# RobustFieldAutonomyLab/Distributional_RL_Navigation

Hardware: AMD Instinct MI355X
Metric: env steps/sec (whole node) at 65 536 envs; IQN grad-steps/sec (higher is better)
Workload: dtype f32; 1 GPU; 65536 envs/GPU + IQN training (act K=32, 8 quantiles, replay 100000, batch 256, 1 grad step(s) every 4 vector steps); envs_per_gpu=65536, n_cores=8, n_obstacles=10, precision=f64, learner=independent, ranks_per_gpu=1, act_variant=2, taus=per_env, resets=under_next_act, launches_per_grad_step=1, ablation=False

## Files before the change

distributional_rl_navigation_amd/_capi.py:

```python
import ctypes as C
import os
import subprocess

_HERE = os.path.dirname(os.path.abspath(__file__))
LIB_PATH = os.path.join(_HERE, "libmarinenav_hip.so")

MAX_CORES, MAX_OBS, NUM_BEAMS, OBS_DIM, NUM_ACTIONS, MAX_STAGES = 8, 10, 11, 26, 9, 8
PRECISION_F64, PRECISION_MIXED = 0, 1
RESET_IN_FRONT, RESET_UNDER_ACT, RESET_OWED = 0, 1, 2
QUERY_VELOCITY_GIVEN, QUERY_VELOCITY_FROM_CURRENT = 0, 1
QUERY_FLAG_COLLISION, QUERY_FLAG_OUTSIDE, QUERY_FLAG_GOAL, QUERY_FLAG_BAD_ENV = 1, 2, 4, 128
INFO_STRINGS = ("normal", "out of boundary", "too long episode", "collision", "reach goal")


class MnParams(C.Structure):
    _fields_ = [
        ("width", C.c_double), ("height", C.c_double), ("core_r", C.c_double), ("v_rel_max", C.c_double),
        ("p", C.c_double), ("v_range", C.c_double * 2), ("obs_r_range", C.c_double * 2), ("clear_r", C.c_double),
        ("goal_dis", C.c_double), ("timestep_penalty", C.c_double), ("collision_penalty", C.c_double),
        ("goal_reward", C.c_double), ("discount", C.c_double), ("min_start_goal_dis", C.c_double),
        ("init_theta", C.c_double), ("init_speed", C.c_double), ("dt", C.c_double), ("robot_r", C.c_double),
        ("max_speed", C.c_double), ("a", C.c_double * 3), ("w", C.c_double * 3), ("sonar_range", C.c_double),
        ("sonar_angle", C.c_double), ("num_cores", C.c_int32), ("num_obs", C.c_int32),
        ("reset_start_and_goal", C.c_int32), ("random_reset_state", C.c_int32), ("set_boundary", C.c_int32),
# ... 71 lines not shown
    ("mn_reset_placement", _i32, [C.c_float, _i32, _i64, _i32, _i32, _i32]),
    ("mn_reset_done_next_act", C.c_int, [_vp, _pf, _vp, C.c_float, _i32, _i32, C.POINTER(_vp), C.POINTER(C.c_uint32), _pi32]),
    ("mn_set_reset_owed_max_rows", C.c_int, [_vp, _i32]),
    ("mn_reset_is_owed", _i32, [_vp]),
    ("mn_reset_join", C.c_int, [_vp, _vp]),
    ("mn_set_reset_under_act_max", C.c_int, [_vp, _i32, C.POINTER(C.c_int64)]),
    ("mn_debug_side_delay_us", C.c_int, [_vp, _i32]),
    ("mn_debug_read", C.c_int, [_vp, _i32, _vp, _i64]),
    ("mn_load_worlds", C.c_int, [_vp, _i32, _i32, _pi32, _pd, _pi32, _pd, _pi32, _pd, _pd, _pd, _pd, _pd, _pd, _pf, _vp]),
    ("mn_get_worlds", C.c_int, [_vp, _i32, _i32, _pi32, _pd, _pi32, _pd, _pi32, _pd, _pd, _pd, _pd, _pd, _pd]),
    ("mn_query_velocity", C.c_int, [_vp, _vp, _i32, _vp, _i64, _vp, _vp]),
    ("mn_query_observation", C.c_int, [_vp, _vp, _i32, _vp, _i32, _i64, _vp, _vp, _vp, _vp]),
    ("mn_get_state", C.c_int, [_vp, _i32, _i32, _pd, _pi32, _pi64]),
    ("mn_set_state", C.c_int, [_vp, _i32, _i32, _pd, _pi32, _pi64]),
    ("mn_state_bytes", _i64, [_vp]),
    ("mn_state_save", C.c_int, [_vp, _vp, _i64, _vp]),
    ("mn_state_load", C.c_int, [_vp, _vp, _i64, _vp]),
    ("mn_enable_obs64", C.c_int, [_vp, _i32]),
    ("mn_get_obs64", C.c_int, [_vp, _i32, _i32, _pd]),
    ("mn_get_reward64", C.c_int, [_vp, _i32, _i32, _pd]),
    ("mn_enable_trajectory", C.c_int, [_vp, _i32]),
    ("mn_get_trajectory", C.c_int, [_vp, _i32, _i32, _i32, _pd]),
    ("mn_set_trajectory_trace", C.c_int, [_vp, _vp, _i32, _i32]),
    ("mn_peek_next_double", C.c_int, [_vp, _i32, _i32, _pd]),
    ("mn_last_done_count", C.c_int, [_vp, _vp, _pi32]),
    ("mn_profile_begin", C.c_int, [_vp, _i32]),
    ("mn_profile_end", C.c_int, [_vp, _vp, _pd, _pi32]),
    ("mn_profile_reset_end", C.c_int, [_vp, _vp, _pd, _pi32]),
    ("mn_iqn_create", C.c_int, [C.POINTER(_vp)]),
    ("mn_iqn_destroy", C.c_int, [_vp]),
    ("mn_iqn_weights_changed", C.c_int, [_vp]),
    ("mn_iqn_set_variant", C.c_int, [_vp, _i32]),
    ("mn_iqn_set_greedy_rows", C.c_int, [_vp, _i32]),
    ("mn_iqn_set_grid", C.c_int, [_vp, _i32]),
    ("mn_iqn_set_tau_mode", C.c_int, [_vp, _i32]),
    ("mn_iqn_set_late_rows", C.c_int, [_vp, _vp, _vp, C.c_uint32, _i32]),
    ("mn_iqn_late_timeouts", C.c_int, [_vp, _vp, C.POINTER(C.c_uint32)]),
    ("mn_iqn_late_timeouts_peek", C.c_int, [_vp, C.POINTER(C.c_uint32)]),
    ("mn_iqn_set_late_bound_ms", C.c_int, [_vp, C.c_double]),
    ("mn_iqn_train_workspace_init", C.c_int, [_vp, _i32, _vp]),
    ("mn_iqn_train_step", C.c_int, [_vp, _vp, _vp, _vp, _vp, _i64, _vp, _vp, _vp, _vp, _vp, _vp, _vp, _vp, _vp, _vp, _vp, _vp, _vp, _vp, _i32, _i32, C.c_float, _i32,
                                    _dbl, _dbl, _dbl, _dbl, _dbl, _vp]),
    ("mn_rollout_policy", C.c_int, [_vp, _i32, _i32, _vp, _vp, _vp, _vp, _vp, _vp, _vp]),
    ("mn_planner_act", C.c_int, [_vp, _i32, _i32, _pd, _pd, _vp, _vp]),
    ("mn_rollout_iqn", C.c_int, [_vp, _vp, C.POINTER(C.c_void_p), _i32, _vp, C.c_float, _i32] + [_vp] * 10),
    ("mn_rollout_iqn_rows", C.c_int, [_vp, _vp, C.POINTER(C.c_void_p), _i32, _vp, C.c_float, _i32] + [_vp] * 12),
    ("mn_rollout_iqn_eval", C.c_int, [_vp, _vp, C.POINTER(C.c_void_p), _i32, _vp, C.c_float, _i32] + [_vp] * 14),
    ("mn_iqn_image_floats", _i32, []),
    ("mn_iqn_export_image", C.c_int, [_vp, C.POINTER(C.c_void_p), _vp, _vp]),
    ("mn_rollout_iqn_groups", C.c_int, [_vp, _vp, _i64, _i32, _i32, _i32] + [_vp] * 14),
    ("mn_rollout_dqn", C.c_int, [_vp, C.POINTER(C.c_void_p), _vp, _i32, _i32] + [_vp] * 8),
    ("mn_dqn_image_floats", C.c_int64, []),
    ("mn_dqn_export_image", C.c_int, [C.POINTER(C.c_void_p), _vp, _vp]),
    ("mn_rollout_dqn_groups", C.c_int, [_vp, _vp, _i64, _i32, _i32, _i32] + [_vp] * 8),
    ("mn_dqn_act", C.c_int, [_vp, C.POINTER(C.c_void_p), _vp, _i32, _vp, _vp, _i32, _vp]),
    ("mn_dqn_train_workspace_floats", C.c_int64, [_i32]),
    ("mn_dqn_train_step", C.c_int, [_vp] * 5 + [_i64] + [_vp] * 11 + [_i32, C.c_float] + [_dbl] * 5 + [_vp]),
    ("mn_dqn_train_steps_workspace_floats", C.c_int64, [_i32, _i32]),
    ("mn_dqn_train_steps", C.c_int, [_vp] * 5 + [_i64] + [_vp] * 11 + [_i32, _i32, C.c_float] + [_dbl] * 5 + [_vp]),
    ("mn_dqn_train_steps_parts", C.c_int, [_vp] * 5 + [_i64] + [_vp] * 11 + [_i32, _i32, C.c_float] + [_dbl] * 5 + [_i32, _vp]),
    ("mn_dqn_group_create", C.c_int, [C.POINTER(MnDqnLearner), _i32, C.POINTER(_vp)]),
    ("mn_dqn_group_destroy", C.c_int, [_vp]),
    ("mn_dqn_group_train_step", C.c_int, [_vp, _i64, _vp, _vp, _vp, _vp, _i32, C.c_float] + [_dbl] * 5 + [_vp]),
    ("mn_dqn_group_train_steps", C.c_int, [_vp, _i64, _vp, _vp, _vp, _vp, _i32, _i32, C.c_float] + [_dbl] * 5 + [_vp]),
    ("mn_iqn_group_create", C.c_int, [C.POINTER(MnIqnLearner), _i32, _i32, C.POINTER(_vp)]),
    ("mn_iqn_group_destroy", C.c_int, [_vp]),
# ... 86 lines not shown
```

distributional_rl_navigation_amd/csrc/iqn_act.hip:

```cpp
#include <hip/hip_runtime.h>
#include <stdint.h>
#include <utility>
#include <vector>

#include "marinenav_hip.h"
#include "mn_internal.h"
#include "iqn_actor_group.h"

#define MN_IQN_VARIANT_DEFAULT 2

namespace {

#include "iqn_act_common.h"
#include "iqn_act_exact.h"
#include "iqn_act_split.h"
#include "iqn_act_tiled.h"
#include "iqn_act_group.h"

using ExactKernel = decltype(&iqn_qvals_kernel<false>);
using SplitKernel = decltype(&sp::iqn_qvals_split_kernel<false>);
using TiledKernel = decltype(&sp::iqn_qvals_tiled_kernel);
struct Form {
    ExactKernel exact;
    SplitKernel split;
    TiledKernel tiled;
    int lds_floats, threads;
    const void *kernel() const { return exact ? (const void *)exact : split ? (const void *)split : (const void *)tiled; }
    size_t lds_bytes() const { return lds_floats * sizeof(float); }
};
enum { F_EXACT, F_EXACT_QUANT, F_SPLIT, F_SPLIT_LATE, F_SPLIT_ROWS, F_SPLIT_LATE_ROWS, F_SPLIT_QUANT, F_SHARED, F_SHARED_QUANT, F_TILED, N_FORMS };
const Form FORMS[N_FORMS] = {
    {iqn_qvals_kernel<false>, nullptr, nullptr, LDS_FLOATS, 512},
    {iqn_qvals_kernel<true>, nullptr, nullptr, LDS_FLOATS, 512},
    {nullptr, sp::iqn_qvals_split_kernel<false>, nullptr, sp::LDS_ACT_FLOATS, 512},
    {nullptr, sp::iqn_qvals_split_kernel<false, false, sp::WAVES, true>, nullptr, sp::LDS_ACT_FLOATS, 512},
    {nullptr, sp::iqn_qvals_split_kernel<false, false, sp::WAVES, false, true>, nullptr, sp::LDS_ACT_FLOATS, 512},
    {nullptr, sp::iqn_qvals_split_kernel<false, false, sp::WAVES, true, true>, nullptr, sp::LDS_ACT_FLOATS, 512},
    {nullptr, sp::iqn_qvals_split_kernel<true>, nullptr, sp::LDS_FLOATS, 512},
    {nullptr, sp::iqn_qvals_split_kernel<false, true, 8>, nullptr, sp::OFF_FB, 512},
    {nullptr, sp::iqn_qvals_split_kernel<true, true, 8>, nullptr, sp::OFF_FB, 512},
    {nullptr, nullptr, sp::iqn_qvals_tiled_kernel, sp::TL_FLOATS, 512},
};

bool load_weights(const float *const *p, IqnWeights *w) {
    if (!p) return false;
    for (int i = 0; i < 14; ++i) if (!p[i]) return false;
    *w = {p[0], p[1], p[2], p[3], p[4], p[5], p[6], p[7], p[8], p[9], p[10], p[11], p[12], p[13]};
    return true;
}

}

struct mn_iqn_ctx {
    int device = -1;
    int n_cu = 0;
    float *packed = nullptr;
    uint32_t *packed_sp = nullptr;
    float *consts_sp = nullptr;
    float *h1_sp = nullptr;
    uint32_t *timg = nullptr;
    float *taux = nullptr;
    template <class Fn> void each_buffer(Fn f) {
        f(packed, OFF_FB); f(packed_sp, sp::OFF_FB); f(consts_sp, sp::N_CONST_BUF); f(h1_sp, sp::H1_FLOATS + 32); f(timg, sp::T_WORDS); f(taux, sp::TA_FLOATS);
    }
    int tau_mode = 0;
    bool dirty = true, dirty_sp = true;
    int variant = MN_IQN_VARIANT_DEFAULT;
    int max_blocks = 0;
    sp::LateRows late = {};
    uint32_t *late_status = nullptr;
    volatile uint32_t *late_status_host = nullptr;
    uint32_t *late_status_host_dev = nullptr;
    uint64_t late_bound_ticks = sp::LATE_BOUND_TICKS;
    std::vector<hipEvent_t> ev;
    int prof_max = 0, prof_n = 0;
    uint32_t *rollout_words = nullptr;
    bool greedy_rows = true;
    uint32_t *rows_buf = nullptr;
    int rows_cap = 0;
};

extern "C" int mn_iqn_set_grid(mn_iqn_ctx *c, int32_t max_workgroups) {
    if (!c || max_workgroups < 0) return MN_ERR_INVALID;
    c->max_blocks = max_workgroups;
    return MN_OK;
}

extern "C" int mn_iqn_create(mn_iqn_ctx **out) {
    if (!out) return MN_ERR_INVALID;
    int dev = 0;
    if (hipGetDevice(&dev) != hipSuccess) return MN_ERR_NO_DEVICE;
    hipDeviceProp_t prop;
    if (hipGetDeviceProperties(&prop, dev) != hipSuccess) return MN_ERR_HIP;
    for (const Form &f : FORMS)
        if (hipFuncSetAttribute(f.kernel(), hipFuncAttributeMaxDynamicSharedMemorySize, (int)f.lds_bytes()) != hipSuccess) return MN_ERR_HIP;
    mn_iqn_ctx *c = new mn_iqn_ctx();
    c->device = dev;
    c->n_cu = prop.multiProcessorCount;
    bool ok = true;
    c->each_buffer([&](auto *&p, size_t count) { ok = ok && hipMalloc(reinterpret_cast<void **>(&p), count * sizeof(*p)) == hipSuccess; });
    if (!ok || hipMemset(c->consts_sp, 0, sp::N_CONST_BUF * sizeof(float)) != hipSuccess || hipDeviceSynchronize() != hipSuccess) {
        c->each_buffer([](auto *p, size_t) { (void)hipFree(p); });
        delete c;
        return MN_ERR_ALLOC;
    }
    *out = c;
    return MN_OK;
}

extern "C" int mn_iqn_destroy(mn_iqn_ctx *c) {
    if (!c) return MN_ERR_INVALID;
    int cur = -1;
    const bool moved = hipGetDevice(&cur) == hipSuccess && cur != c->device;
    if (moved) (void)hipSetDevice(c->device);
    for (hipEvent_t e : c->ev) (void)hipEventDestroy(e);
    c->each_buffer([](auto *p, size_t) { (void)hipFree(p); });
    (void)hipFree(c->late_status);
    (void)hipFree(c->rollout_words);
    (void)hipFree(c->rows_buf);
    if (c->late_status_host) (void)hipHostFree((void *)c->late_status_host);
    if (moved) (void)hipSetDevice(cur);
    delete c;
    return MN_OK;
}

extern "C" int mn_iqn_weights_changed(mn_iqn_ctx *c) {
    if (!c) return MN_ERR_INVALID;
    c->dirty = true;
    c->dirty_sp = true;
    return MN_OK;
}

extern "C" int mn_iqn_set_variant(mn_iqn_ctx *c, int32_t variant) {
    if (!c || (variant != 0 && variant != 2)) return MN_ERR_INVALID;
    c->variant = variant;
    return MN_OK;
}

extern "C" int mn_iqn_set_greedy_rows(mn_iqn_ctx *c, int32_t on) {
    if (!c) return MN_ERR_INVALID;
    c->greedy_rows = on != 0;
    return MN_OK;
}

static int greedy_rows_buffer(mn_iqn_ctx *c, int n, GreedyRows *out) {
    if (n > c->rows_cap) {
        uint32_t *buf = nullptr;
        if (hipMalloc(reinterpret_cast<void **>(&buf), (4 + (size_t)n) * sizeof(uint32_t)) != hipSuccess) return MN_ERR_ALLOC;
        if (hipMemset(buf, 0, 4 * sizeof(uint32_t)) != hipSuccess || hipDeviceSynchronize() != hipSuccess) { (void)hipFree(buf); return MN_ERR_HIP; }
        (void)hipFree(c->rows_buf);
        c->rows_buf = buf;
        c->rows_cap = n;
    }
    *out = GreedyRows{reinterpret_cast<int32_t *>(c->rows_buf + 4), c->rows_buf};
    return MN_OK;
}

extern "C" int mn_iqn_last_greedy_rows(mn_iqn_ctx *c, void *stream, int32_t *list_host, int32_t cap, int32_t *count_out) {
    if (!c || !count_out || cap < 0 || (cap > 0 && !list_host)) return MN_ERR_INVALID;
    *count_out = 0;
    if (!c->rows_buf) return MN_OK;
    if (hipStreamSynchronize((hipStream_t)stream) != hipSuccess) return MN_ERR_HIP;
    uint32_t w[4];
    if (hipMemcpy(w, c->rows_buf, sizeof(w), hipMemcpyDeviceToHost) != hipSuccess) return MN_ERR_HIP;
    const uint32_t count = w[w[2] & 1u];
    if (count > (uint32_t)c->rows_cap) return MN_ERR_HIP;
    *count_out = (int32_t)count;
    const uint32_t k = count < (uint32_t)cap ? count : (uint32_t)cap;
    if (k && hipMemcpy(list_host, c->rows_buf + 4, k * sizeof(int32_t), hipMemcpyDeviceToHost) != hipSuccess) return MN_ERR_HIP;
    return MN_OK;
}

extern "C" int mn_iqn_set_tau_mode(mn_iqn_ctx *c, int32_t mode) {
    if (!c || mode < 0 || mode > 3) return MN_ERR_INVALID;
    c->tau_mode = mode;
    return MN_OK;
}

extern "C" int mn_iqn_profile_begin(mn_iqn_ctx *c, int32_t max_launches) {
    if (!c || max_launches < 0 || max_launches > 65536) return MN_ERR_INVALID;
    while ((int)c->ev.size() < 2 * max_launches) {
        hipEvent_t e;
        if (hipEventCreate(&e) != hipSuccess) return MN_ERR_HIP;
        c->ev.push_back(e);
    }
    c->prof_max = max_launches;
    c->prof_n = 0;
    return MN_OK;
}

extern "C" int mn_iqn_profile_end(mn_iqn_ctx *c, void *stream, double *mean_ms, int32_t *launches) {
    if (!c) return MN_ERR_INVALID;
    if (hipStreamSynchronize((hipStream_t)stream) != hipSuccess) return MN_ERR_HIP;
    double sum = 0.0;
    for (int i = 0; i < c->prof_n; ++i) {
        float ms = 0.f;
        if (hipEventElapsedTime(&ms, c->ev[2 * i], c->ev[2 * i + 1]) != hipSuccess) return MN_ERR_HIP;
        sum += ms;
    }
    if (mean_ms) *mean_ms = c->prof_n ? sum / c->prof_n : 0.0;
    if (launches) *launches = c->prof_n;
    c->prof_max = 0;
    c->prof_n = 0;
    return MN_OK;
}

static int act_grid(const mn_iqn_ctx *c, int n) {
    const int blocks = (n + 7) / 8, cap = c->max_blocks > 0 ? c->max_blocks : c->n_cu;
    return blocks < cap ? blocks : cap;
}

static int draw_blocks(const mn_iqn_ctx *c, long items) {
    const long blocks = (items + 255) / 256;
    return blocks < 8L * c->n_cu ? (int)blocks : 8 * c->n_cu;
}

static bool late_rows_supported(const mn_iqn_ctx *c, int n, bool quantiles) {
    if (c->variant != 2 || c->tau_mode != 0 || quantiles || n <= 0) return false;
    return (long)n <= 64L * 8L * act_grid(c, n);
}

extern "C" int mn_iqn_set_late_rows(mn_iqn_ctx *c, const uint8_t *mask_dev, const uint32_t *flags_dev, uint32_t tick, int32_t n) {
    if (!c) return MN_ERR_INVALID;
    c->late = sp::LateRows{};
    if (!mask_dev && !flags_dev) return MN_OK;
    if (!mask_dev || !flags_dev) return MN_ERR_INVALID;
    if (!late_rows_supported(c, n, false)) return 1;
    if (!c->late_status) {
        uint32_t *st = nullptr;
        void *hp = nullptr, *hd = nullptr;
        if (hipMalloc(reinterpret_cast<void **>(&st), sizeof(uint32_t)) != hipSuccess) return MN_ERR_ALLOC;
        if (hipMemset(st, 0, sizeof(uint32_t)) != hipSuccess || hipHostMalloc(&hp, sizeof(uint32_t), hipHostMallocMapped) != hipSuccess) { (void)hipFree(st); return MN_ERR_ALLOC; }
        *(volatile uint32_t *)hp = 0u;
        if (hipHostGetDevicePointer(&hd, hp, 0) != hipSuccess) { (void)hipFree(st); (void)hipHostFree(hp); return MN_ERR_HIP; }
        c->late_status = st; c->late_status_host = (volatile uint32_t *)hp; c->late_status_host_dev = (uint32_t *)hd;
    }
    c->late = sp::LateRows{mask_dev, flags_dev, tick, c->late_status, c->late_status_host_dev, c->late_bound_ticks};
    return MN_OK;
}

extern "C" int mn_iqn_late_timeouts(mn_iqn_ctx *c, void *stream, uint32_t *out) {
    if (!c || !out) return MN_ERR_INVALID;
// ... 71 lines not shown
    const bool prof = c->prof_n < c->prof_max;
    if (prof) (void)hipEventRecord(c->ev[2 * c->prof_n], s);

    const int pack_blocks = begin_pack(c, w, s);
    if (shared) {
        const int rng_blocks = rng ? draw_blocks(c, (long)n + K_TAUS) : 0;
        hipLaunchKernelGGL(sp::iqn_shared_prep_kernel, dim3(pack_blocks + sp::H1_BLOCKS + rng_blocks), dim3(256), 0, s, w, (const float *)c->consts_sp,
                           c->packed_sp, (const uint64_t *)rng_state_dev, draws_dev, n, rng ? nullptr : taus_dev, cvar, pack_blocks, c->h1_sp);
        if (rng) explore_u_dev = eps > 0.f ? draws_dev + K_TAUS : nullptr;
        taus_dev = nullptr;
        if (f.tiled)
            hipLaunchKernelGGL(sp::iqn_tiled_prep_kernel, dim3(sp::T_PREP_BLOCKS + sp::TA_PREP_BLOCKS), dim3(256), 0, s, w, (const float *)c->consts_sp,
                               (const float *)c->h1_sp, c->timg, c->taux);
    } else if (rng) {
        const int rng_blocks = draw_blocks(c, ((long)n * (K_TAUS + 1) + 3) / 4);
        MnOwedReset owed;
        if (fusable && env && mn_owed_reset_take(env, s, &owed))
            mn_launch_prep_reset(owed, MnPrepLaunch{weights, c->consts_sp, c->packed_sp, pack_blocks != 0, rng_state_dev, draws_dev, n, cvar_row_dev, cvar, eps,
                                                    listed ? actions_dev : nullptr, rows.list, rows.words, 32 * c->n_cu}, s);
        else if (f.split)
            hipLaunchKernelGGL(sp::iqn_split_prep_kernel, dim3(pack_blocks + rng_blocks), dim3(256), 0, s, w, (const float *)c->consts_sp,
                               c->packed_sp, (const uint64_t *)rng_state_dev, draws_dev, n, cvar_row_dev, cvar, pack_blocks, eps, listed ? actions_dev : nullptr,
                               rows);
        else
            hipLaunchKernelGGL(iqn_prep_kernel, dim3(pack_blocks + rng_blocks), dim3(256), 0, s, w, c->packed,
                               (const uint64_t *)rng_state_dev, draws_dev, n, cvar_row_dev, cvar, pack_blocks);
        taus_dev = draws_dev;
        explore_u_dev = eps > 0.f ? draws_dev + (size_t)n * K_TAUS : nullptr;
    } else if (pack_blocks) {
        pack_image(c, w, s);
    }

    const dim3 grid(act_grid(c, n)), block(f.threads);
    if (f.tiled)
        hipLaunchKernelGGL(f.tiled, dim3((n + 255) / 256), block, f.lds_bytes(), s, obs_dev, (const uint32_t *)c->packed_sp, (const uint32_t *)c->timg,
                           (const float *)c->taux, qvals_dev, explore_u_dev, eps, actions_dev, n, rng_state_dev);
    else if (f.split)
        hipLaunchKernelGGL(f.split, grid, block, f.lds_bytes(), s, obs_dev, taus_dev, (const uint32_t *)c->packed_sp, qvals_dev, explore_u_dev, eps,
                           actions_dev, n, rng_state_dev, quantiles_dev, shared ? (const float *)c->h1_sp : nullptr, late, rows);
    else
        hipLaunchKernelGGL(f.exact, grid, block, f.lds_bytes(), s, obs_dev, taus_dev, (const float *)c->packed, qvals_dev, explore_u_dev, eps,
                           actions_dev, n, rng_state_dev, quantiles_dev);

    if (prof) { (void)hipEventRecord(c->ev[2 * c->prof_n + 1], s); ++c->prof_n; }
    return hipGetLastError() == hipSuccess ? MN_OK : MN_ERR_HIP;
}

extern "C" int mn_iqn_refresh(mn_iqn_ctx *c, const float *const *weights, void *stream) {
    IqnWeights w;
    if (!c || !load_weights(weights, &w)) return MN_ERR_INVALID;
    int dev = -1;
    if (hipGetDevice(&dev) != hipSuccess || dev != c->device) return MN_ERR_INVALID;
    if (begin_pack(c, w, (hipStream_t)stream)) pack_image(c, w, (hipStream_t)stream);
    return hipGetLastError() == hipSuccess ? MN_OK : MN_ERR_HIP;
}

int mn_iqn_rollout_image(mn_iqn_ctx *c, const float *const *weights, hipStream_t s, const uint32_t **image, uint32_t **words) {
    if (!c || !weights || !image || !words || c->variant != 2 || c->tau_mode != 0) return MN_ERR_INVALID;
    if (!c->rollout_words) {
        uint32_t *w = nullptr;
        if (hipMalloc(reinterpret_cast<void **>(&w), 2 * sizeof(uint32_t)) != hipSuccess) return MN_ERR_ALLOC;
        if (hipMemset(w, 0, 2 * sizeof(uint32_t)) != hipSuccess || hipDeviceSynchronize() != hipSuccess) { (void)hipFree(w); return MN_ERR_HIP; }
        c->rollout_words = w;
    }
    const int rc = mn_iqn_refresh(c, weights, (void *)s);
    if (rc) return rc;
    *image = c->packed_sp;
// ... 147 lines not shown
```

distributional_rl_navigation_amd/iqn/fused_act.py:

```python
import ctypes as C
import weakref

import torch

from .. import _capi
from ..episodes import EPISODE_TRACES, trace_buffers

_ORDER = ("velocity_encoder", "goal_encoder", "sensor_encoder", "cos_embedding", "hidden_layer", "hidden_layer_2", "output_layer")


def _p(t):
    return C.c_void_p(t.data_ptr()) if t is not None else None


def _params(net):
    mods = net._modules
    out = []
    for name in _ORDER:
        ps = mods[name]._parameters
        out.append(ps["weight"]); out.append(ps["bias"])
    return out


class ActContext:

    def __init__(self, device):
        self.device = torch.device(device)
        h = C.c_void_p()
        with torch.cuda.device(self.device):
            rc = _capi.lib().mn_iqn_create(C.byref(h))
        if rc:
            raise _capi.MarineNavHipError(f"mn_iqn_create failed ({rc})")
        self.h = h
        self._sig = None
        self.variant = self.DEFAULT_VARIANT
        self.tau_mode = 0
        self.greedy_rows = True
        self._ptrs = (C.c_void_p * 14)()
        self._fin = weakref.finalize(self, _capi.lib().mn_iqn_destroy, h)

    def __deepcopy__(self, memo):
        return None

    def __reduce__(self):
        return (type(None), ())

    def weights(self, net):
        ps = _params(net)
        sig = tuple((t.data_ptr(), t._version) for t in ps)
        if sig != self._sig:
            for i, t in enumerate(ps):
                assert t.is_cuda and t.is_contiguous() and t.dtype == torch.float32
                self._ptrs[i] = t.data_ptr()
            self._sig = sig
            self.invalidate()
        return self._ptrs

    def invalidate(self):
        _capi.lib().mn_iqn_weights_changed(self.h)

    DEFAULT_VARIANT = 2

    def set_variant(self, variant):
        rc = _capi.lib().mn_iqn_set_variant(self.h, int(variant))
        if rc:
            raise _capi.MarineNavHipError(f"mn_iqn_set_variant failed ({rc})")
        self.variant = int(variant)

    def set_greedy_rows(self, on):
        if bool(on) == self.greedy_rows:
            return
        rc = _capi.lib().mn_iqn_set_greedy_rows(self.h, int(bool(on)))
        if rc:
            raise _capi.MarineNavHipError(f"mn_iqn_set_greedy_rows failed ({rc})")
        self.greedy_rows = bool(on)

    def set_tau_mode(self, mode):
        if int(mode) == self.tau_mode:
            return
        rc = _capi.lib().mn_iqn_set_tau_mode(self.h, int(mode))
        if rc:
            raise _capi.MarineNavHipError(f"mn_iqn_set_tau_mode failed ({rc})")
        self.tau_mode = int(mode)

    def set_grid(self, max_workgroups):
        rc = _capi.lib().mn_iqn_set_grid(self.h, int(max_workgroups))
        if rc:
            raise _capi.MarineNavHipError(f"mn_iqn_set_grid failed ({rc})")
        self.__dict__.pop("_late_ok", None)

    def refresh(self, net):
        stream = _capi.stream_ptr(self.device)
        rc = _capi.lib().mn_iqn_refresh(self.h, self.weights(net), stream)
        if rc:
            raise _capi.MarineNavHipError(f"mn_iqn_refresh failed ({rc})")

    def profile_begin(self, max_launches):
        rc = _capi.lib().mn_iqn_profile_begin(self.h, int(max_launches))
        if rc:
            raise _capi.MarineNavHipError(f"mn_iqn_profile_begin failed ({rc})")

    def profile_end(self):
        ms, nl = C.c_double(), C.c_int32()
        stream = _capi.stream_ptr(self.device)
        rc = _capi.lib().mn_iqn_profile_end(self.h, stream, C.byref(ms), C.byref(nl))
        if rc:
            raise _capi.MarineNavHipError(f"mn_iqn_profile_end failed ({rc})")
        return ms.value, nl.value
# ... 253 lines not shown
```

include/marinenav_hip.h:

```cpp
#ifndef MARINENAV_HIP_H
#define MARINENAV_HIP_H

#include <stdint.h>

#ifdef __cplusplus
extern "C" {
#endif

#define MN_MAX_CORES 8
#define MN_MAX_OBS 10
#define MN_NUM_BEAMS 11
#define MN_OBS_DIM 26
#define MN_NUM_ACTIONS 9
#define MN_MAX_STAGES 8

typedef enum mn_status {
    MN_OK = 0,
    MN_ERR_INVALID = -1,
    MN_ERR_HIP = -2,
    MN_ERR_NO_DEVICE = -3,
    MN_ERR_ALLOC = -4,
    MN_ERR_PEER = -5
} mn_status;

// ... 125 lines not shown
                         uint8_t *flags_dev, void *stream);

int mn_get_state(mn_handle *h, int32_t first_env, int32_t count, double *state, int32_t *episode_timesteps,
                 int64_t *total_timesteps);
int mn_set_state(mn_handle *h, int32_t first_env, int32_t count, const double *state,
                 const int32_t *episode_timesteps, const int64_t *total_timesteps);

int64_t mn_state_bytes(const mn_handle *h);
int mn_state_save(mn_handle *h, void *blob_dev, int64_t bytes, void *stream);
int mn_state_load(mn_handle *h, const void *blob_dev, int64_t bytes, void *stream);

int mn_enable_obs64(mn_handle *h, int32_t on);
int mn_get_obs64(mn_handle *h, int32_t first_env, int32_t count, double *out);
int mn_get_reward64(mn_handle *h, int32_t first_env, int32_t count, double *out);

int mn_enable_trajectory(mn_handle *h, int32_t max_substeps);
int mn_get_trajectory(mn_handle *h, int32_t first_env, int32_t count, int32_t n_substeps, double *out);
int mn_set_trajectory_trace(mn_handle *h, double *traj_trace_dev, int32_t n_steps, int32_t n_substeps);

int mn_peek_next_double(mn_handle *h, int32_t first_env, int32_t count, double *out);

int mn_last_done_count(mn_handle *h, void *stream, int32_t *out);

int mn_profile_begin(mn_handle *h, int32_t max_launches);
int mn_profile_reset_end(mn_handle *h, void *stream, double *mean_ms, int32_t *launches);
int mn_profile_end(mn_handle *h, void *stream, double *mean_ms, int32_t *launches);

typedef struct mn_iqn_ctx mn_iqn_ctx;
int mn_iqn_create(mn_iqn_ctx **out);
int mn_iqn_destroy(mn_iqn_ctx *c);
int mn_iqn_weights_changed(mn_iqn_ctx *c);
int mn_iqn_set_variant(mn_iqn_ctx *c, int32_t variant);
int mn_iqn_set_greedy_rows(mn_iqn_ctx *c, int32_t on);
int mn_iqn_set_tau_mode(mn_iqn_ctx *c, int32_t mode);
int mn_iqn_last_greedy_rows(mn_iqn_ctx *c, void *stream, int32_t *list_host, int32_t cap, int32_t *count_out);
int mn_iqn_set_late_rows(mn_iqn_ctx *c, const uint8_t *mask_dev, const uint32_t *flags_dev, uint32_t tick, int32_t n);
int mn_iqn_late_timeouts(mn_iqn_ctx *c, void *stream, uint32_t *out);
int mn_iqn_late_timeouts_peek(mn_iqn_ctx *c, uint32_t *out);
int mn_iqn_set_late_bound_ms(mn_iqn_ctx *c, double ms);
int mn_probe_mfma_clock(double target_ms, double *out, void *stream);
int mn_iqn_set_grid(mn_iqn_ctx *c, int32_t max_workgroups);
int mn_iqn_refresh(mn_iqn_ctx *c, const float *const *weights, void *stream);

int mn_iqn_act(mn_iqn_ctx *c, const float *obs_dev, const float *taus_dev, const float *const *weights, float *qvals_dev,
               const float *explore_u_dev, float eps, int32_t *actions_dev, float *quantiles_dev, int32_t n,
               int32_t num_taus, void *stream);

int mn_iqn_act_rng(mn_iqn_ctx *c, const float *obs_dev, const float *const *weights, uint64_t *rng_state_dev,
                   float *draws_dev, const float *cvar_row_dev, float cvar, float eps, int32_t *actions_dev,
                   float *qvals_dev, float *quantiles_dev, int32_t n, int32_t num_taus, void *stream);
int mn_iqn_act_rng_env(mn_iqn_ctx *c, mn_handle *env, const float *obs_dev, const float *const *weights, uint64_t *rng_state_dev,
                       float *draws_dev, const float *cvar_row_dev, float cvar, float eps, int32_t *actions_dev,
                       float *qvals_dev, float *quantiles_dev, int32_t n, int32_t num_taus, void *stream);
int mn_rollout_iqn(mn_handle *h, mn_iqn_ctx *ctx, const float *const *weights, int32_t n_steps, uint64_t *rng_state_dev, float cvar,
                   int32_t adaptive, float *obs_dev, float *obs_trace_dev, float *reward_trace_dev, uint8_t *done_trace_dev,
                   uint8_t *info_trace_dev, int32_t *action_trace_dev, float *cvar_trace_dev, float *q_trace_dev, int32_t *steps_run_dev,
                   void *stream);
int mn_rollout_iqn_rows(mn_handle *h, mn_iqn_ctx *ctx, const float *const *weights, int32_t n_steps, uint64_t *rng_state_dev, float cvar,
                        int32_t adaptive, const float *cvar_row_dev, const uint8_t *adaptive_row_dev, float *obs_dev, float *obs_trace_dev,
                        float *reward_trace_dev, uint8_t *done_trace_dev, uint8_t *info_trace_dev, int32_t *action_trace_dev, float *cvar_trace_dev,
                        float *q_trace_dev, int32_t *steps_run_dev, void *stream);
int mn_rollout_iqn_eval(mn_handle *h, mn_iqn_ctx *ctx, const float *const *weights, int32_t n_steps, uint64_t *rng_state_dev, float cvar,
                        int32_t adaptive, const float *cvar_row_dev, const uint8_t *adaptive_row_dev, float *obs_dev, float *obs_trace_dev,
                        float *reward_trace_dev, uint8_t *done_trace_dev, uint8_t *info_trace_dev, int32_t *action_trace_dev, float *cvar_trace_dev,
                        float *q_trace_dev, float *quantiles_trace_dev, float *taus_trace_dev, int32_t *steps_run_dev, void *stream);

// ... 164 lines not shown
```

Measured before the change: 910.5 million env steps/s.

## Add few-rows IQN act kernel with register ring-prefetched weights

Adds a separate act kernel for the greedy-rows split form, used when the expected number of greedy rows ((1-eps)*n) is at most a threshold (default 256). Each block handles one row at a time with two waves. Weight fragments stream from global memory through an eight-deep register ring that is prefetched and interleaved with the MFMA stages, instead of the full-device tiled/split path. The aim is lower latency when only a few rows need network evaluation, such as early high-epsilon exploration. The cost is a large new hand-scheduled kernel, and it only triggers at small greedy-row counts, so at 65536 envs with low eps it may rarely run.

```diff
diff --git a/distributional_rl_navigation_amd/_capi.py b/distributional_rl_navigation_amd/_capi.py
--- a/distributional_rl_navigation_amd/_capi.py
+++ b/distributional_rl_navigation_amd/_capi.py
@@ -127,6 +127,8 @@
     ("mn_iqn_weights_changed", C.c_int, [_vp]),
     ("mn_iqn_set_variant", C.c_int, [_vp, _i32]),
     ("mn_iqn_set_greedy_rows", C.c_int, [_vp, _i32]),
+    ("mn_iqn_set_few_rows_max", C.c_int, [_vp, _i32]),
+    ("mn_iqn_few_rows_launches", C.c_int, [_vp, C.POINTER(C.c_int64)]),
     ("mn_iqn_set_grid", C.c_int, [_vp, _i32]),
     ("mn_iqn_set_tau_mode", C.c_int, [_vp, _i32]),
     ("mn_iqn_set_late_rows", C.c_int, [_vp, _vp, _vp, C.c_uint32, _i32]),
diff --git a/distributional_rl_navigation_amd/csrc/iqn_act.hip b/distributional_rl_navigation_amd/csrc/iqn_act.hip
--- a/distributional_rl_navigation_amd/csrc/iqn_act.hip
+++ b/distributional_rl_navigation_amd/csrc/iqn_act.hip
@@ -14,6 +14,7 @@
 #include "iqn_act_common.h"
 #include "iqn_act_exact.h"
 #include "iqn_act_split.h"
+#include "iqn_act_few.h"
 #include "iqn_act_tiled.h"
 #include "iqn_act_group.h"
 
@@ -78,6 +79,8 @@
     bool greedy_rows = true;
     uint32_t *rows_buf = nullptr;
     int rows_cap = 0;
+    int few_rows_max = MN_IQN_FEW_ROWS_MAX_DEFAULT;
+    int64_t few_launches = 0;
 };
 
 extern "C" int mn_iqn_set_grid(mn_iqn_ctx *c, int32_t max_workgroups) {
@@ -143,6 +146,18 @@
     return MN_OK;
 }
 
+extern "C" int mn_iqn_set_few_rows_max(mn_iqn_ctx *c, int32_t rows) {
+    if (!c) return MN_ERR_INVALID;
+    c->few_rows_max = rows;
+    return MN_OK;
+}
+
+extern "C" int mn_iqn_few_rows_launches(mn_iqn_ctx *c, int64_t *out) {
+    if (!c || !out) return MN_ERR_INVALID;
+    *out = c->few_launches;
+    return MN_OK;
+}
+
 static int greedy_rows_buffer(mn_iqn_ctx *c, int n, GreedyRows *out) {
     if (n > c->rows_cap) {
         uint32_t *buf = nullptr;
@@ -208,6 +223,17 @@
 static int act_grid(const mn_iqn_ctx *c, int n) {
     const int blocks = (n + 7) / 8, cap = c->max_blocks > 0 ? c->max_blocks : c->n_cu;
     return blocks < cap ? blocks : cap;
+}
+
+static bool few_rows(const mn_iqn_ctx *c, const Form &f, int n, float eps) {
+    if (&f != &FORMS[F_SPLIT_ROWS] || c->few_rows_max < 0) return false;
+    return (1.0 - (eps < 1.f ? (double)eps : 1.0)) * (double)n <= (double)c->few_rows_max;
+}
+
+static int few_grid(const mn_iqn_ctx *c, int n) {
+    const int cap = c->max_blocks > 0 ? c->max_blocks : c->n_cu, want = c->few_rows_max < 1 ? 1 : c->few_rows_max;
+    const int blocks = want < cap ? want : cap;
+    return blocks < n ? blocks : n;
 }
 
 static int draw_blocks(const mn_iqn_ctx *c, long items) {
@@ -345,7 +371,11 @@
     }
 
     const dim3 grid(act_grid(c, n)), block(f.threads);
-    if (f.tiled)
+    if (few_rows(c, f, n, eps)) {
+        ++c->few_launches;
+        hipLaunchKernelGGL(sp::iqn_act_few_kernel, dim3(few_grid(c, n)), dim3(64 * sp::FEW_WAVES), 0, s, obs_dev, taus_dev, (const uint32_t *)c->packed_sp, actions_dev,
+                           n, rng_state_dev, rows);
+    } else if (f.tiled)
         hipLaunchKernelGGL(f.tiled, dim3((n + 255) / 256), block, f.lds_bytes(), s, obs_dev, (const uint32_t *)c->packed_sp, (const uint32_t *)c->timg,
                            (const float *)c->taux, qvals_dev, explore_u_dev, eps, actions_dev, n, rng_state_dev);
     else if (f.split)
diff --git a/distributional_rl_navigation_amd/csrc/iqn_act_few.h b/distributional_rl_navigation_amd/csrc/iqn_act_few.h
--- /dev/null
+++ b/distributional_rl_navigation_amd/csrc/iqn_act_few.h
@@ -0,0 +1,294 @@
+
+namespace sp {
+
+constexpr int FEW_WAVES = 2;
+constexpr int FEW_DEPTH = 8;
+constexpr int FEW_PRE = 4;
+constexpr int FEW_MID = 4;
+
+constexpr int FEW_L1 = 0, FEW_L2 = 1, FEW_B2 = 2, FEW_L3 = 3, FEW_B3 = 4, FEW_W4 = 5;
+struct FewGrp { int kind, a, b; };
+constexpr FewGrp few_group(int gi) {
+    int k = 0;
+    for (int t = 0; t < 4; ++t, ++k) if (k == gi) return {FEW_L1, t, 0};
+    for (int B = 0; B < KB2 - 1; ++B) {
+        for (int h = 0; h < 2; ++h, ++k) if (k == gi) return {FEW_L2, B, h};
+        for (int t = 2 * B + 4; t < 2 * B + 6 && t < T1; ++t, ++k) if (k == gi) return {FEW_L1, t, 0};
+    }
+    for (int h = 0; h < 2; ++h, ++k) if (k == gi) return {FEW_L2, KB2 - 1, h};
+    if (k++ == gi) return {FEW_B2, 0, 0};
+    for (int kb = 0; kb < 2; ++kb)
+        for (int h = 0; h < 2; ++h, ++k) if (k == gi) return {FEW_L3, kb, h};
+    if (k++ == gi) return {FEW_B3, 0, 0};
+    if (k++ == gi) return {FEW_W4, 0, 0};
+    return {-1, 0, 0};
+}
+constexpr int few_index(int kind, int a, int b) {
+    for (int gi = 0; gi < 64; ++gi) {
+        const FewGrp g = few_group(gi);
+        if (g.kind < 0) break;
+        if (g.kind == kind && g.a == a && g.b == b) return gi;
+    }
+    return -1;
+}
+constexpr int FEW_GROUPS = few_index(FEW_W4, 0, 0) + 1;
+static_assert(FEW_GROUPS == T1 + 2 * KB2 + 4 + 3, "every weight operand of a row once, and the three groups of f32 constants");
+constexpr int few_unit(int gi, int j) {
+    const FewGrp g = few_group(gi);
+    if (g.kind == FEW_L1) return j < 4 ? W1_U4 + (4 * g.a + j) * 64 : (OFF_B1 >> 2) + 4 * g.a;
+    if (g.kind == FEW_L2) return W2_U4 + (((2 * g.b + (j >> 1)) * KB2 + g.a) * 2 + (j & 1)) * 64;
+    if (g.kind == FEW_L3) return W3_U4 + (((2 * g.b + (j >> 1)) * 2 + g.a) * 2 + (j & 1)) * 64;
+    if (g.kind == FEW_B2) return (OFF_B2 >> 2) + 4 * j;
+    if (g.kind == FEW_B3) return (OFF_B3 >> 2) + 4 * j;
+    return (OFF_W4 >> 2) + j * 64;
+}
+static_assert(OFF_B1 % 4 == 0 && OFF_B2 % 4 == 0 && OFF_B3 % 4 == 0 && OFF_W4 % 4 == 0, "16-byte aligned blocks");
+
+typedef u32x4 FewRing[FEW_DEPTH][5];
+
+typedef const __attribute__((address_space(1))) char *FewImage;
+struct FewOff { uint32_t lane, group; FewImage image; };
+__device__ __forceinline__ u32x4 few_ld(const FewOff &o, int unit, uint32_t off) {
+    return *reinterpret_cast<const __attribute__((address_space(1))) u32x4 *>(o.image + 16 * unit + off);
+}
+template <int GI>
+__device__ __forceinline__ void few_load(FewRing &ring, const FewOff &o) {
+    if constexpr (GI < FEW_GROUPS) {
+        constexpr FewGrp G = few_group(GI);
+        constexpr int s = GI % FEW_DEPTH;
+        constexpr bool by_group = G.kind == FEW_B2 || G.kind == FEW_B3;
+        static_for<4>([&](auto J_) {
+            constexpr int j = decltype(J_)::value;
+            ring[s][j] = few_ld(o, few_unit(GI, j), by_group ? o.group : o.lane);
+        });
+        if constexpr (G.kind == FEW_L1) ring[s][4] = few_ld(o, few_unit(GI, 4), o.group);
+    }
+}
+
+template <int B>
+__device__ __forceinline__ void few_stage(FewRing &ring, const FewOff &o, const f32x4 *__restrict__ fbv,
+                                          const f16x8 (&cbh)[2], const f16x8 (&cbl)[2], const f16x8 bh, const f16x8 bl, f32x4 (&acc2)[4],
+                                          f32x4 (&accW)[2], const f32x4 (&accR)[2], f16x8 &bhN, f16x8 &blN) {
+    constexpr int NTI_W = (B + 2 < KB2) ? ntiles_of(B + 2) : 0;
+    constexpr int NTI_R = (B + 1 >= 0 && B + 1 < KB2) ? ntiles_of(B + 1) : 0;
+    constexpr int N_L2 = B >= 0 ? 12 : 0, N_L1 = 6 * NTI_W, N_MIX = 2 * (N_L2 < N_L1 ? N_L2 : N_L1), NM = N_L2 + N_L1;
+    constexpr int N_UNIT = NTI_R * 2;
+    f32x4 fv[2];
+#pragma unroll
+    for (int ti = 0; ti < NTI_R; ++ti) fv[ti] = fbv[4 * (2 * (B + 1) + ti)];
+    const f16x2 zero2 = {(_Float16)0.f, (_Float16)0.f};
+    f16x2 hP[4] = {zero2, zero2, zero2, zero2}, lP[4] = {zero2, zero2, zero2, zero2};
+    __builtin_amdgcn_sched_barrier(0);
+    static_for<NM>([&](auto M_) {
+        constexpr int m = decltype(M_)::value;
+        constexpr bool is_l2 = m < N_MIX ? (m % 2 == 0) : (N_L2 > N_L1);
+        constexpr int idx = m < N_MIX ? m / 2 : m - N_MIX / 2;
+        if constexpr (is_l2) {
+            constexpr int p = idx / 4, mt = idx % 4;
+            constexpr int gi = few_index(FEW_L2, B, mt / 2), s = gi % FEW_DEPTH;
+            const f16x8 ah = __builtin_bit_cast(f16x8, ring[s][2 * (mt & 1)]), al = __builtin_bit_cast(f16x8, ring[s][2 * (mt & 1) + 1]);
+            acc2[mt] = mf(p == 0 ? al : ah, p == 1 ? bl : bh, acc2[mt]);
+            if constexpr (p == 2 && (mt & 1)) few_load<gi + FEW_DEPTH>(ring, o);
+        } else {
+            constexpr int kb = idx / (3 * NTI_W), p = (idx % (3 * NTI_W)) / NTI_W, ti = idx % NTI_W;
+            constexpr int gi = few_index(FEW_L1, 2 * (B + 2) + ti, 0), s = gi % FEW_DEPTH;
+            const f16x8 ah = __builtin_bit_cast(f16x8, ring[s][2 * kb]), al = __builtin_bit_cast(f16x8, ring[s][2 * kb + 1]);
+            accW[ti] = mf(p == 0 ? al : ah, p == 1 ? cbl[kb] : cbh[kb], (kb == 0 && p == 0) ? __builtin_bit_cast(f32x4, ring[s][4]) : accW[ti]);
+            if constexpr (kb == 1 && p == 2) few_load<gi + FEW_DEPTH>(ring, o);
+        }
+#pragma unroll
+        for (int u = 0; u < N_UNIT; ++u) {
+            if ((u + 1) * NM / (N_UNIT + 1) == m) {
+                const int ti = u / 2, pr = u % 2;
+                float x0 = relu1(accR[ti][2 * pr]), x1 = relu1(accR[ti][2 * pr + 1]);
+                x0 *= fv[ti][2 * pr]; x1 *= fv[ti][2 * pr + 1];
+                const f16x2 hcur = cvt_pair(x0, x1);
+                const float r0 = residual_lo32(x0, hcur), r1 = residual_hi32(x1, hcur);
+                hP[2 * ti + pr] = hcur;
+                lP[2 * ti + pr] = cvt_pair(r0, r1);
+            }
+        }
+        __builtin_amdgcn_sched_barrier(0);
+    });
+    if (N_UNIT > 0) {
+        bhN = cat4(hP[0], hP[1], hP[2], hP[3]);
+        blN = cat4(lP[0], lP[1], lP[2], lP[3]);
+    }
+}
+
+__device__ __forceinline__ void few_tail(FewRing &ring, const FewOff &o, float c2, float S, const f16x8 bh, const f16x8 bl,
+                                         f32x4 (&acc2)[4], f32x4 (&acc3)[4]) {
+    constexpr int sB2 = few_index(FEW_B2, 0, 0) % FEW_DEPTH;
+#pragma unroll
+    for (int mt = 0; mt < 4; ++mt) acc3[mt] = (f32x4){0.f, 0.f, 0.f, 0.f};
+    f32x4 sb[4];
+    f16x2 hP[2][4], lP[2][4];
+    f16x8 b3h[2], b3l[2];
+    __builtin_amdgcn_sched_barrier(0);
+    static_for<36>([&](auto M_) {
+        constexpr int m = decltype(M_)::value;
+        if constexpr (m < 12) {
+            constexpr int half = m / 6, q = m % 6, p = q / 2, mt = 2 * half + q % 2;
+            constexpr int gi = few_index(FEW_L2, KB2 - 1, half), s = gi % FEW_DEPTH;
+            const f16x8 ah = __builtin_bit_cast(f16x8, ring[s][2 * (mt & 1)]), al = __builtin_bit_cast(f16x8, ring[s][2 * (mt & 1) + 1]);
+            acc2[mt] = mf(p == 0 ? al : ah, p == 1 ? bl : bh, acc2[mt]);
+            if constexpr (p == 2 && (mt & 1)) few_load<gi + FEW_DEPTH>(ring, o);
+        } else {
+            constexpr int kb = (m - 12) / 12, q = (m - 12) % 12, p = q / 4, mt = q % 4;
+            constexpr int gi = few_index(FEW_L3, kb, mt / 2), s = gi % FEW_DEPTH;
+            const f16x8 ah = __builtin_bit_cast(f16x8, ring[s][2 * (mt & 1)]), al = __builtin_bit_cast(f16x8, ring[s][2 * (mt & 1) + 1]);
+            acc3[mt] = mf(p == 0 ? al : ah, p == 1 ? b3l[kb] : b3h[kb], acc3[mt]);
+            if constexpr (p == 2 && (mt & 1)) few_load<gi + FEW_DEPTH>(ring, o);
+        }
+        if constexpr (m == 5) {
+#pragma unroll
+            for (int t = 0; t < 4; ++t) sb[t] = __builtin_bit_cast(f32x4, ring[sB2][t]) * S;
+            few_load<few_index(FEW_B2, 0, 0) + FEW_DEPTH>(ring, o);
+        }
+#pragma unroll
+        for (int u = 0; u < 8; ++u) {
+            if ((u < 4 ? 6 + u : 8 + u) == m) {
+                const int half = u / 4, ti = (u % 4) / 2, pr = u % 2, t = 2 * half + ti;
+                const float t0 = relu1(fmaf(acc2[t][2 * pr], c2, sb[t][2 * pr])), t1 = relu1(fmaf(acc2[t][2 * pr + 1], c2, sb[t][2 * pr + 1]));
+                const f16x2 hcur = cvt_pair(t0, t1);
+                float r0, r1;
+                residual_pair(t0, t1, hcur, r0, r1);
+                hP[half][2 * ti + pr] = hcur;
+                lP[half][2 * ti + pr] = cvt_pair(r0, r1);
+                if (u % 4 == 3) {
+                    b3h[half] = cat4(hP[half][0], hP[half][1], hP[half][2], hP[half][3]);
+                    b3l[half] = cat4(lP[half][0], lP[half][1], lP[half][2], lP[half][3]);
+                }
+            }
+        }
+        __builtin_amdgcn_sched_barrier(0);
+    });
+}
+
+__global__ __launch_bounds__(64 * FEW_WAVES, 2) void iqn_act_few_kernel(const float *__restrict__ obs, const float *__restrict__ taus,
+                                                                        const uint32_t *__restrict__ packed, int32_t *__restrict__ actions, int n,
+                                                                        uint64_t *__restrict__ rng_state, const GreedyRows rows) {
+    __shared__ __attribute__((aligned(16))) float s_fb[FEW_WAVES * F];
+    __shared__ __attribute__((aligned(16))) float s_h3[16 * 64];
+    const int tid = threadIdx.x, wave = __builtin_amdgcn_readfirstlane(tid >> 6);
+    const int lane = tid & 63, g = lane >> 4;
+    const int col = lane & 15;
+    const float *pf = reinterpret_cast<const float *>(packed);
+    const f32x4 *pv = reinterpret_cast<const f32x4 *>(packed);
+    const uint32_t wd[3] = {rows.words[0], rows.words[1], rows.words[2]};
+    const int pos0 = blockIdx.x;
+    const int row0 = rows.list[pos0 < n ? pos0 : n - 1];
+    __builtin_amdgcn_sched_barrier(0);
+    const char *image = reinterpret_cast<const char *>(packed);
+    FewOff o = {16u * (uint32_t)lane, 16u * (uint32_t)g, (FewImage)image};
+    asm volatile("" : "+v"(o.lane), "+v"(o.group));
+    FewRing ring;
+    static_for<FEW_PRE>([&](auto I_) { few_load<decltype(I_)::value>(ring, o); });
+    const float c1 = pf[OFF_CST + 0], c2 = pf[OFF_CST + 1], c3 = pf[OFF_CST + 2];
+    const float a2 = pf[OFF_CST + 3], d2 = pf[OFF_CST + 4], a3 = pf[OFF_CST + 5], d3 = pf[OFF_CST + 6];
+    const float b4c = pf[OFF_B4 + col];
+    const uint32_t slot = wd[2] & 1u, count = slot ? wd[1] : wd[0];
+    const int n_rows = count < (uint32_t)n ? (int)count : n;
+    if (pos0 == 0 && tid == 0) {
+        if (rng_state) rng_state[1] += 1;
+        rows.words[3] = slot ^ 1u;
+    }
+    if (pos0 >= n_rows) return;
+
+    const int fb_f = wave * F + lane;
+    const f32x4 *fbv = reinterpret_cast<const f32x4 *>(s_fb) + ((wave * F) >> 2) + g;
+    const float hk0 = 4.0f * (float)g;
+    const auto eval_row = [&](int row) __attribute__((always_inline)) {
+        row = __builtin_amdgcn_readfirstlane(row);
+        int enc_w = (OFF_WS >> 2) + lane;
+        int enc_f = OFF_BND + lane;
+        float hk = hk0;
+        asm volatile("" : "+v"(o.lane), "+v"(o.group), "+v"(enc_w), "+v"(enc_f), "+v"(hk), "+s"(image));
+        o.image = (FewImage)image;
+        if ((unsigned)row < (unsigned)n) {
+            const float tau = taus[(size_t)row * K_TAUS + 16 * wave + col];
+            const float *orow = obs + (size_t)row * OBS;
+            float ov[28];
+#pragma unroll
+            for (int i = 0; i < 28; ++i) ov[i] = i < OBS ? orow[i] : 0.f;
+            static_for<FEW_MID - FEW_PRE>([&](auto I_) { few_load<FEW_PRE + decltype(I_)::value>(ring, o); });
+            f16x8 cbh[2], cbl[2];
+#pragma unroll
+            for (int kb = 0; kb < 2; ++kb) {
+                f16x2 h[4], l[4];
+#pragma unroll
+                for (int p = 0; p < 4; ++p)
+                    split2(__builtin_amdgcn_cosf(tau * (hk + (16.0f * kb + 0.5f * (2 * p)))),
+                           __builtin_amdgcn_cosf(tau * (hk + (16.0f * kb + 0.5f * (2 * p + 1)))), h[p], l[p]);
+                cbh[kb] = cat4(h[0], h[1], h[2], h[3]);
+                cbl[kb] = cat4(l[0], l[1], l[2], l[3]);
+            }
+            EncState st;
+            static_for<N_ENC_SUB>([&](auto I_) { enc_substep<decltype(I_)::value>(pf, pv, enc_w, enc_f, lane, ov, st); });
+            const EnvScale sc = env_scale(st.bnd, a2, d2, a3, d3);
+            store_features(s_fb, fb_f, lane, st, sc.S1 * c1);
+            __builtin_amdgcn_wave_barrier();
+            asm volatile("s_waitcnt lgkmcnt(0)" ::: "memory");
+            static_for<FEW_DEPTH - FEW_MID>([&](auto I_) { few_load<FEW_MID + decltype(I_)::value>(ring, o); });
+
+            f32x4 acc2[4], acc3[4], accA[2], accB[2];
+#pragma unroll
+            for (int mt = 0; mt < 4; ++mt) acc2[mt] = (f32x4){0.f, 0.f, 0.f, 0.f};
+            f16x8 bhA, blA, bhB, blB;
+            bhA = blA = bhB = blB = __builtin_bit_cast(f16x8, (u32x4){0u, 0u, 0u, 0u});
+            few_stage<-2>(ring, o, fbv, cbh, cbl, bhB, blB, acc2, accA, accB, bhB, blB);
+            few_stage<-1>(ring, o, fbv, cbh, cbl, bhB, blB, acc2, accB, accA, bhA, blA);
+            few_stage<0>(ring, o, fbv, cbh, cbl, bhA, blA, acc2, accA, accB, bhB, blB);
+            few_stage<1>(ring, o, fbv, cbh, cbl, bhB, blB, acc2, accB, accA, bhA, blA);
+            few_stage<2>(ring, o, fbv, cbh, cbl, bhA, blA, acc2, accA, accB, bhB, blB);
+            few_stage<3>(ring, o, fbv, cbh, cbl, bhB, blB, acc2, accB, accA, bhA, blA);
+            few_stage<4>(ring, o, fbv, cbh, cbl, bhA, blA, acc2, accA, accB, bhB, blB);
+            few_stage<5>(ring, o, fbv, cbh, cbl, bhB, blB, acc2, accB, accA, bhA, blA);
+            few_tail(ring, o, c2 * sc.r21, sc.S2, bhA, blA, acc2, acc3);
+
+            constexpr int sB3 = few_index(FEW_B3, 0, 0) % FEW_DEPTH, sW4 = few_index(FEW_W4, 0, 0) % FEW_DEPTH;
+            const float c3e = c3 * sc.r32;
+            f32x4 hv[4];
+#pragma unroll
+            for (int mt = 0; mt < 4; ++mt) {
+                const f32x4 sb = __builtin_bit_cast(f32x4, ring[sB3][mt]) * sc.S3;
+                hv[mt] = relu4s(fma4(acc3[mt], c3e, sb));
+            }
+            if (wave == 1) {
+#pragma unroll
+                for (int i = 0; i < 16; ++i) s_h3[i * 64 + lane] = hv[i >> 2][i & 3];
+            }
+            __syncthreads();
+            if (wave == 0) {
+                float hs[16];
+#pragma unroll
+                for (int i = 0; i < 16; ++i) hs[i] = hv[i >> 2][i & 3] + s_h3[i * 64 + lane];
+                row_sum16_x16(hs);
+                float part = 0.f;
+#pragma unroll
+                for (int mt = 0; mt < 4; ++mt) {
+                    const f32x4 a = __builtin_bit_cast(f32x4, ring[sW4][mt]);
+#pragma unroll
+                    for (int r = 0; r < 4; ++r) part = fmaf(a[r], hs[4 * mt + r], part);
+                }
+                part = sum_rows4(part);
+                const float qv = part * (sc.invS3 * (1.0f / K_TAUS)) + b4c;
+                float best = __builtin_bit_cast(float, __builtin_amdgcn_readlane(__builtin_bit_cast(int, qv), 0));
+                int arg = 0;
+#define SP_ARG(a) { const float v = __builtin_bit_cast(float, __builtin_amdgcn_readlane(__builtin_bit_cast(int, qv), a)); if (v > best) { best = v; arg = a; } }
+                SP_ARG(1) SP_ARG(2) SP_ARG(3) SP_ARG(4) SP_ARG(5) SP_ARG(6) SP_ARG(7) SP_ARG(8)
+#undef SP_ARG
+                if (lane == 0) actions[row] = arg;
+            }
+        }
+    };
+    eval_row(row0);
+    for (int pos = pos0 + (int)gridDim.x; pos < n_rows; pos += (int)gridDim.x) {
+        __syncthreads();
+        const int row = rows.list[pos];
+        static_for<FEW_PRE>([&](auto I_) { few_load<decltype(I_)::value>(ring, o); });
+        eval_row(row);
+    }
+}
+
+}
diff --git a/distributional_rl_navigation_amd/iqn/fused_act.py b/distributional_rl_navigation_amd/iqn/fused_act.py
--- a/distributional_rl_navigation_amd/iqn/fused_act.py
+++ b/distributional_rl_navigation_amd/iqn/fused_act.py
@@ -36,6 +36,7 @@
         self.variant = self.DEFAULT_VARIANT
         self.tau_mode = 0
         self.greedy_rows = True
+        self.few_rows_max = self.FEW_ROWS_MAX_DEFAULT
         self._ptrs = (C.c_void_p * 14)()
         self._fin = weakref.finalize(self, _capi.lib().mn_iqn_destroy, h)
 
@@ -74,6 +75,23 @@
         if rc:
             raise _capi.MarineNavHipError(f"mn_iqn_set_greedy_rows failed ({rc})")
         self.greedy_rows = bool(on)
+
+    FEW_ROWS_MAX_DEFAULT = 256
+    FEW_ROWS_ALWAYS = 2 ** 31 - 1
+
+    def set_few_rows_max(self, rows=None):
+        rows = self.FEW_ROWS_MAX_DEFAULT if rows is None else int(rows)
+        rc = _capi.lib().mn_iqn_set_few_rows_max(self.h, rows)
+        if rc:
+            raise _capi.MarineNavHipError(f"mn_iqn_set_few_rows_max failed ({rc})")
+        self.few_rows_max = rows
+
+    def few_rows_launches(self):
+        out = C.c_int64()
+        rc = _capi.lib().mn_iqn_few_rows_launches(self.h, C.byref(out))
+        if rc:
+            raise _capi.MarineNavHipError(f"mn_iqn_few_rows_launches failed ({rc})")
+        return out.value
 
     def set_tau_mode(self, mode):
         if int(mode) == self.tau_mode:
diff --git a/include/marinenav_hip.h b/include/marinenav_hip.h
--- a/include/marinenav_hip.h
+++ b/include/marinenav_hip.h
@@ -181,6 +181,11 @@
 int mn_iqn_weights_changed(mn_iqn_ctx *c);
 int mn_iqn_set_variant(mn_iqn_ctx *c, int32_t variant);
 int mn_iqn_set_greedy_rows(mn_iqn_ctx *c, int32_t on);
+#ifndef MN_IQN_FEW_ROWS_MAX_DEFAULT
+#define MN_IQN_FEW_ROWS_MAX_DEFAULT 256
+#endif
+int mn_iqn_set_few_rows_max(mn_iqn_ctx *c, int32_t rows);
+int mn_iqn_few_rows_launches(mn_iqn_ctx *c, int64_t *out);
 int mn_iqn_set_tau_mode(mn_iqn_ctx *c, int32_t mode);
 int mn_iqn_last_greedy_rows(mn_iqn_ctx *c, void *stream, int32_t *list_host, int32_t cap, int32_t *count_out);
 int mn_iqn_set_late_rows(mn_iqn_ctx *c, const uint8_t *mask_dev, const uint32_t *flags_dev, uint32_t tick, int32_t n);
```

After: 993.3 million env steps/s (median of 6 runs). +9.1%, better.
